# afombravo/2FAST2Q

Hardware: AMD Instinct MI355X
Metric: Mreads/sec matched (150 bp, 20 bp feature, m=1) (higher is better)
Workload: dtype u64 (2-bit packed bases) / u8 qualities

## Files before the change

### 2fast2q_amd/csrc/f2q_count_kernels.h

```cpp
#pragma once

#define F2Q_HIST_MAX 24576u
#define F2Q_HIST_RANGE 38912u

__device__ __forceinline__ unsigned long long wave_sum(unsigned long long v)
{
    for (int o = 32; o > 0; o >>= 1) v += __shfl_down(v, o, 64);
    return v;
}

__device__ __forceinline__ void flush_stats(const Accum &acc, unsigned long long st[5], unsigned long long *lds8,
                                            unsigned long long *slab_row)
{
    const uint32_t lane = threadIdx.x & 63u;
    if (threadIdx.x < 8) lds8[threadIdx.x] = 0;
    __syncthreads();
    for (int k = 0; k < 5; k++) {
        unsigned long long v = wave_sum(st[k]);
        if (lane == 0 && v) atomicAdd(&lds8[k], v);
    }
    __syncthreads();
    if (threadIdx.x < 5) {
        unsigned long long v = lds8[threadIdx.x];
        if (slab_row) gpw(slab_row)[threadIdx.x] = v;
// ... 426 lines not shown
    typedef uint32_t v2 __attribute__((ext_vector_type(2)));
    const v2 v = *reinterpret_cast<const v2 *>(p);
    return U2{v.x, v.y};
}

__device__ __forceinline__ uint32_t lt_count_inc(uint32_t slot) { return 1u << ((slot & 1u) << 4); }
__device__ __forceinline__ uint32_t lt_count_add(uint32_t *cnt, uint32_t bucket, uint32_t inc)
{
    return atomicAdd(&cnt[bucket], inc);
}
__device__ __forceinline__ bool lt_count_passed(uint32_t old, uint32_t inc) { return ((old >> (inc >> 12)) & 0xFFFFu) == 0x7FFFu; }
__device__ __forceinline__ bool lt_count_maybe_passed(uint32_t old_or) { return (old_or & 0x40004000u) != 0u; }
__device__ __forceinline__ void lt_count_handoff(uint32_t *cnt, uint32_t bucket, uint32_t inc, const Accum &acc, const LtDesc &lt)
{
    atomicSub(&cnt[bucket], inc << 15);
    acc_add(&acc.counts[gp(lt.feat_of)[2u * bucket + (inc >> 16)]], 0x8000ull);
}
__device__ __forceinline__ void lt_count(uint32_t *cnt, uint32_t slot, const Accum &acc, const LtDesc &lt)
{
    const uint32_t bucket = slot >> 1, inc = lt_count_inc(slot);
    if (lt_count_passed(lt_count_add(cnt, bucket, inc), inc)) lt_count_handoff(cnt, bucket, inc, acc, lt);
}

template <int NQ, int NB, bool NEAR, bool A20, bool MW = false>
__global__ __launch_bounds__(F2Q_LT_THREADS) void k_count_fixed4_lds(const RunDev *__restrict__ runp,
                                                                     const LibDev *__restrict__ libp, PackedBlock pb,
                                                                     Accum acc)
{
    extern __shared__ uint32_t lt_smem[];
    constexpr uint32_t NT = NEAR ? 2u : 1u;
    uint32_t *tg = lt_smem;
// ... 1149 lines not shown
    __syncthreads();
    typedef uint32_t v4 __attribute__((ext_vector_type(4)));
    const uint64_t n4 = n_slots / 4;
    const auto hb = (const v4 F2Q_GLOBAL *)hit_buf;
    for (uint64_t i = (uint64_t)part * 1024u + threadIdx.x; i < n4; i += (uint64_t)n_parts * 1024u) {
        const v4 v = hb[i];
        const uint32_t e[4] = {v.x - f0, v.y - f0, v.z - f0, v.w - f0};
#pragma unroll
        for (int k = 0; k < 4; k++) if (e[k] < fn) atomicAdd(&rh[e[k]], 1u);
    }
    __syncthreads();
    auto row = (uint32_t F2Q_GLOBAL *)slab + (uint64_t)part * nf + f0;
    for (uint32_t i = threadIdx.x; i < fn; i += 1024u) row[i] = rh[i];
}

#define F2Q_RED_SPLIT 8u
__global__ __launch_bounds__(256) void k_reduce_slabs(const uint32_t *__restrict__ slab, uint32_t n_rows, uint32_t nf,
                                                       unsigned long long *__restrict__ counts,
                                                       const unsigned long long *__restrict__ stat_slab, uint32_t n_stat_rows,
                                                       unsigned long long *__restrict__ stats)
{
    __shared__ unsigned long long part[256];
    if (blockIdx.x == 0 && blockIdx.y == 0 && stat_slab) {
        const uint32_t k = threadIdx.x & 7u, sub = threadIdx.x >> 3;
        unsigned long long sv = 0;
        if (k < 5) for (uint32_t w = sub; w < n_stat_rows; w += 32u) sv += stat_slab[(uint64_t)w * 8u + k];
        part[threadIdx.x] = sv;
        __syncthreads();
        if (threadIdx.x < 5) {
            unsigned long long tot = 0;
            for (uint32_t q = 0; q < 32u; q++) tot += part[q * 8u + threadIdx.x];
            if (tot) atomicAdd(&stats[threadIdx.x], tot);
        }
        __syncthreads();
    }
    const uint32_t fx = threadIdx.x & 63u, ry = threadIdx.x >> 6;
    const uint32_t f = blockIdx.x * 64u + fx;
    unsigned long long sum = 0;
    if (f < nf) {
        const uint32_t step = F2Q_RED_SPLIT * 4u;
#pragma unroll 8
        for (uint32_t w = blockIdx.y * 4u + ry; w < n_rows; w += step) sum += slab[(uint64_t)w * nf + f];
    }
    part[threadIdx.x] = sum;
    __syncthreads();
    if (ry == 0 && f < nf) {
        sum = part[fx] + part[64 + fx] + part[128 + fx] + part[192 + fx];
        if (sum) atomicAdd(&counts[f], sum);
    }
}

struct RawBlock {
    uint64_t n;
    uint64_t first_index;
    const uint8_t *raw;
    const unsigned long long *off;
    const unsigned long long *qoff;
    const uint32_t *len, *qlen, *index;
    const uint32_t *len1, *qlen1;
    const unsigned long long *hdr_umi;
};

#define F2Q_GEN_THREADS 64
// ... 46 lines not shown
```

### 2fast2q_amd/csrc/f2q_device.h

```cpp
#pragma once
#include <stdint.h>

#ifndef F2Q_HD
#ifdef __HIPCC__
#define F2Q_HD __host__ __device__ __forceinline__
#else
#define F2Q_HD inline
#endif
#endif

#define F2Q_DEV_MAX_ITER 16
#define F2Q_ANCHOR_MAX 128
#define F2Q_MAX_PIECES 8
#define F2Q_REG_MAXLEN 31
#define F2Q_TILE 256
#define F2Q_LEN_SKIP 0xFFFFu
#define F2Q_LEN_FLAG 0x8000u
#define F2Q_LEN_CASE 0x4000u
#define F2Q_LEN_MASK 0x3FFFu

namespace f2q {

#if defined(__HIP_DEVICE_COMPILE__)
#define F2Q_GLOBAL __attribute__((address_space(1)))
// ... 100 lines not shown
    const uint64_t *tab_keys;
    const uint32_t *tab_idx;
    const uint8_t *feat_bytes;
    const uint32_t *feat_off;
    const uint32_t *irr_ids;
    LenGroup grp[F2Q_REG_MAXLEN + 1];
};

struct Accum {
    unsigned long long *counts;
    unsigned long long *stats;
    uint32_t *slab;
    unsigned long long *stat_slab;
    unsigned long long *stamp;
    uint32_t *hit_buf;
};

struct EcDev {
    unsigned long long *slots;
    uint32_t mask;
    uint32_t max_entries;
    unsigned long long *ent_off;
    uint32_t *ent_len;
    unsigned long long *ent_count;
    unsigned long long *ent_first;
    uint32_t *arena;
    unsigned long long arena_words;
    unsigned long long *ctr;
    unsigned long long *k64_slots;
    unsigned long long *k64_count;
// ... 2484 lines not shown
```

### 2fast2q_amd/csrc/f2q_lib.hip

```cpp
#include <hip/hip_runtime.h>
#include <stdio.h>
#include <stdlib.h>
#include <string.h>
#include <zlib.h>

#include <algorithm>
#include <atomic>
#include <string>
#include <chrono>
#include <condition_variable>
#include <deque>
#include <functional>
#include <map>
#include <memory>
#include <unordered_map>
#include <mutex>
#include <thread>
#include <vector>

#include "f2q_device.h"
#include "f2q_host.h"
#include "f2q_synth.h"
#include "f2q_reader.h"

// ... 33 lines not shown
    RunDev *run_d = nullptr;
    PackPlan plan{};
    int n_mate1 = 0;
    bool rc2 = false;
    bool have_lib = false;
    HostIndex ix;
    LibDev lib_h{};
    LibDev *lib_d = nullptr;
    std::vector<void *> lib_allocs;
    uint64_t *guide_keys_d = nullptr;
    std::vector<uint64_t> synth_keys;
    uint64_t *synth_keys_d = nullptr;
    uint32_t synth_glen = 0;
    unsigned long long *acc_d = nullptr;
    uint64_t acc_n = 0;
    uint32_t *slab_d = nullptr;
    size_t slab_n = 0;
    unsigned long long *stat_slab_d = nullptr;
    size_t stat_slab_n = 0;
    uint32_t *hit_buf_d = nullptr;
    size_t hit_buf_n = 0;
    EcDev ec{};
    std::vector<void *> ec_allocs;
    std::vector<void *> ec_allocs64;
    std::vector<void *> ec_allocs_ctr;
    hipStream_t aux_stream = nullptr;
    hipEvent_t ev_aux0 = nullptr, ev_aux1 = nullptr;
    bool aux_busy = false;
    uint64_t ec_slots = 0;
    EcHot hot{};
// ... 247 lines not shown
        L.gk.fw = gk_fw; L.gk.fwoff = gk_fwoff;
    }
    L.tab_keys = tk; L.tab_idx = ti; L.feat_bytes = fb; L.feat_off = fo; L.irr_ids = ir;
    if (guide_keys) *guide_keys = gk;
    LibDev *ld;
    if ((rc = dev_upload(c, &L, 1, &ld, owner))) return rc;
    *lib_d = ld;
    HIPC(c, hipStreamSynchronize(c->stream));
    return F2Q_OK;
}
static int upload_lib(f2q_ctx *c) { return upload_index(c, c->ix, c->lib_h, &c->lib_d, c->lib_allocs, &c->guide_keys_d); }

static int alloc_acc(f2q_ctx *c, uint64_t n_features)
{
    if (c->acc_d) { (void)hipFree(c->acc_d); c->acc_d = nullptr; }
    c->acc_n = n_features + 5;
    HIPC(c, hipMalloc((void **)&c->acc_d, c->acc_n * sizeof(unsigned long long)));
    HIPC(c, hipMemsetAsync(c->acc_d, 0, c->acc_n * sizeof(unsigned long long), c->stream));
    HIPC(c, hipStreamSynchronize(c->stream));
    return F2Q_OK;
}

extern "C" int f2q_create(const f2q_params *p, f2q_ctx **out)
{
    if (!p || !out) return fail(nullptr, F2Q_EINVAL, "null argument");
    *out = nullptr;
    int ndev = 0;
    hipError_t e = hipGetDeviceCount(&ndev);
    if (e != hipSuccess || ndev < 1)
        return fail(nullptr, F2Q_ENODEVICE, std::string("no HIP device: ") + hipGetErrorString(e));
    if (p->device < 0 || p->device >= ndev) return fail(nullptr, F2Q_EINVAL, "device ordinal out of range");
    if (p->mode != 0 && p->mode != 1) return fail(nullptr, F2Q_EINVAL, "mode must be 0 (C) or 1 (EC)");
    f2q_ctx *c = new f2q_ctx();
    c->prm = *p;
// ... 191 lines not shown
    if (c->aux_stream) (void)hipStreamSynchronize(c->aux_stream);
    free_all(c, c->lib_allocs); free_all(c, c->ec_allocs); free_all(c, c->ec_allocs64); free_all(c, c->ec_allocs_ctr); free_all(c, c->hot_allocs);
    free_all(c, c->asg_lib_allocs); free_all(c, c->asg_allocs);
    if (c->trace && c->umi.on) fprintf(stderr, "[f2q trace] UMI set: %llu slots, %llu rehashes\n", (unsigned long long)c->umi.n_slots, (unsigned long long)c->umi.rehashes);
    umi_drop(c);
    demux_drop(c);
    strand_drop(c);
    if (c->trace && c->parts.on) fprintf(stderr, "[f2q trace] recombinant set: %llu slots, %llu rehashes\n", (unsigned long long)c->parts.n_slots, (unsigned long long)c->parts.rehashes);
    parts_drop(c);
    free_all(c, c->stagger.allocs);
    if (c->asg_acc_d) (void)hipFree(c->asg_acc_d);
    if (c->defer_d) (void)hipFree(c->defer_d);
    for (auto &kv : c->dev_idle) (void)hipFree(kv.second);
    c->dev_idle.clear(); c->dev_size.clear();
    if (c->acc_d) (void)hipFree(c->acc_d);
    if (c->synth_keys_d) (void)hipFree(c->synth_keys_d);
    if (c->slab_d) (void)hipFree(c->slab_d);
    if (c->stat_slab_d) (void)hipFree(c->stat_slab_d);
    if (c->hit_buf_d) (void)hipFree(c->hit_buf_d);
    if (c->pt_s.streams) (void)hipFree(c->pt_s.streams);
    if (c->pt_s.cnt) (void)hipFree(c->pt_s.cnt);
    if (c->pt_stat_d) (void)hipFree(c->pt_stat_d);
    if (c->pt_slab0_d) (void)hipFree(c->pt_slab0_d);
    if (c->pt_slab1_d) (void)hipFree(c->pt_slab1_d);
    if (c->run_d) (void)hipFree(c->run_d);
    if (c->ev_a) (void)hipEventDestroy(c->ev_a);
    if (c->ev_b) (void)hipEventDestroy(c->ev_b);
    if (c->ev_k0) (void)hipEventDestroy(c->ev_k0);
    if (c->ev_k1) (void)hipEventDestroy(c->ev_k1);
    for (hipEvent_t e : c->q_ev) (void)hipEventDestroy(e);
// ... 37 lines not shown
    if (c->demux.on) { demux_drop(c); if ((rc = demux_alloc(c))) return rc; }
    if (c->strand.mode) { strand_drop(c); if ((rc = strand_alloc(c))) return rc; }
    if (c->parts.on && (rc = parts_install(c, seqs ? seqs : "", offs, n))) return rc;
    if (c->stagger.n) HIPC(c, hipMemsetAsync(c->stagger.dev.hist, 0, 2 * ((size_t)c->stagger.n + 1) * sizeof(unsigned long long), c->stream));
    c->plan.inband_n = (c->plan.fast_fixed || c->plan.fast_anchor) && c->ix.n_irregular == 0;
    if (c->plan.fast_anchor && c->plan.multi_pair && c->prm.mode == 0 && c->run_h.n_iter == 2 && c->lib_h.pw.ok) { c->plan.inband_n = true; c->plan.n_only = true; }
    if (c->ix.n_irregular && !c->plan.multi_pair) c->plan.fast_anchor = false;
    c->have_lib = true;
    return F2Q_OK;
}

extern "C" int f2q_reset_counts(f2q_ctx *c)
{
    if (!c) return F2Q_EINVAL;
    HIPC(c, hipSetDevice(c->device));
    HIPC(c, hipMemsetAsync(c->acc_d, 0, c->acc_n * sizeof(unsigned long long), c->stream));
    if (c->prm.mode == 1) {
        if (c->aux_stream) HIPC(c, hipStreamSynchronize(c->aux_stream));
        c->aux_busy = false;
        free_all(c, c->ec_allocs); free_all(c, c->ec_allocs64); free_all(c, c->ec_allocs_ctr);
        memset(&c->ec, 0, sizeof c->ec); c->ec_slots = 0; c->hot_valid = false; c->ec_learned = 0;
    }
    if (c->umi.on && c->umi.dev.umis) if (int rc = umi_clear(c)) return rc;
    if (c->demux.on && c->demux.dev.matrix) if (int rc = demux_clear(c)) return rc;
    if (c->strand.mode && c->strand.dev.rev_counts) HIPC(c, hipMemsetAsync(c->strand.dev.rev_counts, 0, c->strand.words * sizeof(unsigned long long), c->stream));
    if (c->parts.on && c->parts.dev.counts) if (int rc = parts_clear(c)) return rc;
    if (c->stagger.n) HIPC(c, hipMemsetAsync(c->stagger.dev.hist, 0, 2 * ((size_t)c->stagger.n + 1) * sizeof(unsigned long long), c->stream));
    c->reads_seen = 0;
    c->ec_gen++;
    return F2Q_OK;
}

extern "C" int f2q_set_read_base(f2q_ctx *c, uint64_t first_read_index)
{
    if (!c) return F2Q_EINVAL;
    c->reads_seen = first_read_index;
    return F2Q_OK;
}

extern "C" int f2q_read_counts(f2q_ctx *c, int64_t *counts, int64_t stats[5])
{
    if (!c) return F2Q_EINVAL;
    HIPC(c, hipSetDevice(c->device));
    std::vector<unsigned long long> h(c->acc_n);
    HIPC(c, hipMemcpyAsync(h.data(), c->acc_d, c->acc_n * sizeof(unsigned long long), hipMemcpyDeviceToHost, c->stream));
    HIPC(c, hipStreamSynchronize(c->stream));
    if (counts) for (uint64_t i = 0; i + 5 < c->acc_n; i++) counts[i] = (int64_t)h[i];
    if (stats) for (int k = 0; k < 5; k++) stats[k] = (int64_t)h[c->acc_n - 5 + k];
    return F2Q_OK;
}

extern "C" int f2q_counts_device_ptr(f2q_ctx *c, void **dptr, uint64_t *n_int64)
{
    if (!c || !dptr || !n_int64) return F2Q_EINVAL;
    *dptr = c->acc_d; *n_int64 = c->acc_n;
    return F2Q_OK;
}

static const char *const STAGGER_NO_UMI = "a stagger context (f2q_set_stagger) takes no UMIs: the two are not combined";
static const char *const STRAND_NO_UMI = "a context with a strand mode (f2q_set_strand: rev / both) takes no UMIs: the two are not combined";
static const char *const PARTS_NO_UMI = "a parts context (f2q_set_parts) takes no UMIs: the two are not combined";
static const char *const DEMUX_NO_UMI = "a demultiplexing context (f2q_set_sample_barcodes) takes no UMIs: the two are not combined";
static void umi_enable(f2q_ctx *c)
{
    c->umi.on = true;
    { const char *e = getenv("F2Q_UMI_SLOTS"); if (e && atol(e) > 0) { c->umi.min_slots = 2; while (c->umi.min_slots < (uint64_t)atol(e) && c->umi.min_slots < (1ull << 32)) c->umi.min_slots <<= 1; } }
    c->force_general = true;
    c->plan.fast_fixed = false; c->plan.fast_anchor = false; c->plan.multi = false; c->plan.multi_pair = false;
    c->plan.inband_n = false; c->plan.n_only = false;
// ... 443 lines not shown
    if (zero) HIPC(c, hipMemsetAsync(*buf, 0, want * sizeof(T), c->stream));
    have = want;
    return F2Q_OK;
}
static int slab_rows(f2q_ctx *c, size_t rows, size_t stat_rows, Accum &acc)
{
    int rc;
    if ((rc = grow_buf(c, &c->slab_d, c->slab_n, std::max<size_t>(rows * c->lib_h.n_features, 1), false))) return rc;
    if ((rc = grow_buf(c, &c->stat_slab_d, c->stat_slab_n, stat_rows * 8, false))) return rc;
    acc.slab = c->slab_d; acc.stat_slab = c->stat_slab_d;
    return F2Q_OK;
}
static int reduce_slabs(f2q_ctx *c, const Accum &acc, uint32_t rows, uint32_t stat_rows, uint32_t &launches)
{
    const uint32_t nf = c->lib_h.n_features;
    hipLaunchKernelGGL(k_reduce_slabs, dim3(std::max<uint32_t>(1u, (nf + 63) / 64), F2Q_RED_SPLIT), dim3(256), 0, c->stream,
                       c->slab_d, rows, nf, acc.counts, c->stat_slab_d, stat_rows, acc.stats);
    HIPC(c, hipGetLastError());
    launches++;
    return F2Q_OK;
}
static bool same_q(const RunDev &r) { return r.thr_up == r.thr && r.thr_down == r.thr; }

template <int N> using int_c = std::integral_constant<int, N>;
template <bool WIDE = false, class F>
static void anchored_geom(int nw, int kb, bool sameq, F &&f)
{
    if constexpr (WIDE) {
        if (nw == 10) return f(int_c<10>(), int_c<3>(), std::false_type());
    }
    auto by_kb = [&](auto NW) {
        auto by_sq = [&](auto KB) { if (sameq) f(NW, KB, std::true_type()); else f(NW, KB, std::false_type()); };
        if (kb == 0) by_sq(int_c<0>()); else if (kb == 1) by_sq(int_c<1>()); else by_sq(int_c<3>());
    };
// ... 66 lines not shown
    launches++;
    return lds && nf ? reduce_slabs(c, acc, grid, grid, launches) : F2Q_OK;
}

static int launch_anchor_lds(f2q_ctx *c, const PackedBlock &pb, Accum &acc, uint32_t &launches)
{
    const uint32_t groups = (pb.n_tiles + F2Q_ALT_GROUPS - 1) / F2Q_ALT_GROUPS;
    uint32_t grid = std::min<uint32_t>(groups, (uint32_t)c->n_cu);
    if (c->lt_max_wgs) grid = std::min<uint32_t>(grid, c->lt_max_wgs);
    const bool near = c->run_h.miss > 0;
    const size_t shmem = ((near ? 2u : 1u) * (size_t)F2Q_LT_SLOTS + F2Q_LT_BUCKETS) * 4;
    int rc = slab_rows(c, grid, grid, acc);
    if (rc) return rc;
    anchored_geom(pb.planar_nw, c->plan.kb, true, [&](auto NW, auto KB, auto) {
        auto kern = near ? k_count_anchor_lt<NW, KB, true, true> : k_count_anchor_lt<NW, KB, true, false>;
        (void)hipFuncSetAttribute((const void *)kern, hipFuncAttributeMaxDynamicSharedMemorySize, (int)shmem);
        hipLaunchKernelGGL(kern, dim3(grid), dim3(F2Q_ALT_THREADS), shmem, c->stream, c->run_d, c->lib_d, pb, acc);
    });
    HIPC(c, hipGetLastError());
    launches++;
    return reduce_slabs(c, acc, grid, grid, launches);
}

static int launch_extract_fixed(f2q_ctx *c, const PackedBlock &pb, Accum &acc, uint32_t &launches)
{
    const uint32_t wgs = (pb.n_tiles + F2Q_V2_WAVES - 1) / F2Q_V2_WAVES;
    const uint32_t grid = std::min<uint32_t>(wgs, (uint32_t)c->n_cu * 4u);
    hipLaunchKernelGGL(k_extract_fixed4, dim3(grid), dim3(F2Q_V2_THREADS), 0, c->stream, c->run_d, c->ec, pb, acc, c->reads_seen);
    HIPC(c, hipGetLastError());
    launches++;
    return F2Q_OK;
}

// ... 33 lines not shown
    int rc;
    if ((rc = grow_buf(c, &c->pt_s.streams, c->pt_streams_n, (size_t)grid1 * P * cap, false))) return rc;
    if ((rc = grow_buf(c, &c->pt_s.cnt, c->pt_cnt_n, (size_t)grid1 * P, false))) return rc;
    if ((rc = grow_buf(c, &c->pt_slab0_d, c->pt_slab0_n, (size_t)grid2 * std::max<uint32_t>(pt.max_part, 1u), true))) return rc;
    if ((rc = grow_buf(c, &c->pt_slab1_d, c->pt_slab1_n, (size_t)n_slots1, true))) return rc;
    if ((rc = grow_buf(c, &c->pt_stat_d, c->pt_stat_n, (size_t)rows * 8, true))) return rc;
    PartScratch ps = c->pt_s;
    ps.cap = cap; ps.n_wg1 = grid1;
    Accum a1 = acc, a2 = acc;
    a1.stat_slab = c->pt_stat_d; a2.stat_slab = a1.stat_slab + (size_t)grid1 * 8;
    const FixedVariant fv = fixed_variant(c, fixed_geom(c->run_h));
    const bool near = c->run_h.miss > 0;
    const size_t shmem1 = (size_t)pw * P * F2Q_PS_RING * 8 + (size_t)(pw + 1) * P * 4;
    const size_t shmem2 = ((size_t)F2Q_LT_SLOTS + F2Q_LT_BUCKETS) * 4 + (near ? (size_t)cw * (F2Q_PC_RING * 8 + F2Q_PC_VIA * 4) : 0);
    auto kern2 = near ? k_part_count<true> : k_part_count<false>;
    (void)hipFuncSetAttribute((const void *)kern2, hipFuncAttributeMaxDynamicSharedMemorySize, (int)shmem2);
    for (uint32_t t0 = 0; t0 < pb.n_tiles; t0 += chunk_tiles) {
        const uint32_t t1 = std::min<uint32_t>(pb.n_tiles, t0 + chunk_tiles);
        auto scatter = [&](auto PW) {
            auto k1 = fv == FV_A20 ? k_part_scatter<5, 2, true, PW> : fv == FV_SPEC52 ? k_part_scatter<5, 2, false, PW> : k_part_scatter<0, 0, false, PW>;
            (void)hipFuncSetAttribute((const void *)k1, hipFuncAttributeMaxDynamicSharedMemorySize, (int)shmem1);
            hipLaunchKernelGGL(k1, dim3(grid1), dim3(64 * PW), shmem1, c->stream, c->run_d, c->lib_d, pb, a1, ps, t0, t1);
        };
        if (pw == 16) scatter(int_c<16>()); else if (pw == 8) scatter(int_c<8>()); else scatter(int_c<4>());
        HIPC(c, hipGetLastError());
        hipLaunchKernelGGL(kern2, dim3(grid2), dim3(64 * cw), shmem2, c->stream, c->run_d, c->lib_d, a2, ps, c->pt_slab0_d, c->pt_slab1_d);
        HIPC(c, hipGetLastError());
        launches += 2;
    }
    hipLaunchKernelGGL(k_part_reduce, dim3(std::max<uint32_t>(1u, (nf + 63) / 64)), dim3(256), 0, c->stream, c->lib_d, c->pt_slab0_d, K,
                       near ? c->pt_slab1_d : (uint32_t *)nullptr, acc.counts, c->pt_stat_d, rows, acc.stats);
    HIPC(c, hipGetLastError());
    launches++;
    return F2Q_OK;
}

template <bool MW>
static auto fixed_lds_kernel(bool near, FixedVariant fv)
{
    if (near) return fv == FV_A20 ? k_count_fixed4_lds<5, 2, true, true, MW> : fv == FV_SPEC52 ? k_count_fixed4_lds<5, 2, true, false, MW> : k_count_fixed4_lds<0, 0, true, false, MW>;
    return fv == FV_A20 ? k_count_fixed4_lds<5, 2, false, true, MW> : fv == FV_SPEC52 ? k_count_fixed4_lds<5, 2, false, false, MW> : k_count_fixed4_lds<0, 0, false, false, MW>;
}
static int launch_fixed_lds(f2q_ctx *c, const PackedBlock &pb, Accum &acc, uint32_t &launches, bool mw)
{
    const uint32_t wgs = (pb.n_tiles + F2Q_LT_WAVES - 1) / F2Q_LT_WAVES;
    const uint32_t grid = std::min<uint32_t>(wgs, c->lt_max_wgs ? std::min<uint32_t>(c->lt_max_wgs, (uint32_t)c->n_cu) : (uint32_t)c->n_cu);
    const bool near = c->run_h.miss > 0;
    const size_t shmem = ((near ? 2u : 1u) * (size_t)F2Q_LT_SLOTS + F2Q_LT_BUCKETS) * 4;
    const FixedVariant fv = fixed_variant(c, mw ? fixed_geom_at(0, c->run_h.n_iter * c->run_h.length, c->run_h.thr) : fixed_geom(c->run_h));
    auto kern = mw ? fixed_lds_kernel<true>(near, fv) : fixed_lds_kernel<false>(near, fv);
    int rc = slab_rows(c, grid, grid, acc);
    if (rc) return rc;
    (void)hipFuncSetAttribute((const void *)kern, hipFuncAttributeMaxDynamicSharedMemorySize, (int)shmem);
    hipLaunchKernelGGL(kern, dim3(grid), dim3(F2Q_LT_THREADS), shmem, c->stream, c->run_d, c->lib_d, pb, acc);
    HIPC(c, hipGetLastError());
    launches++;
    return reduce_slabs(c, acc, grid, grid, launches);
}

static int launch_fixed_packed(f2q_ctx *c, const PackedBlock &pb, Accum &acc, uint32_t &launches)
{
    const uint32_t nf = c->lib_h.n_features;
    const bool lds = nf <= F2Q_HIST_MAX;
    const uint32_t wgs = (pb.n_tiles + F2Q_V2_WAVES - 1) / F2Q_V2_WAVES;
    uint32_t grid = std::min<uint32_t>(wgs, (uint32_t)c->n_cu * 2u);
    if (c->lt_max_wgs) grid = std::min<uint32_t>(grid, c->lt_max_wgs);
    const size_t shmem = (size_t)F2Q_V2_WAVES * F2Q_V2_QCAP * 12 + (lds ? (size_t)nf * 4 : (size_t)F2Q_V2_WAVES * F2Q_V2_QCAP * 4);
    const bool spec52 = fixed_variant(c, fixed_geom(c->run_h)) != FV_GENERIC;
    auto kern = lds ? (spec52 ? k_count_fixed4<true, 5, 2> : k_count_fixed4<true, 0, 0>)
                    : (spec52 ? k_count_fixed4<false, 5, 2> : k_count_fixed4<false, 0, 0>);
    const uint32_t n_ranges = lds ? 1u : (nf + F2Q_HIST_RANGE - 1) / F2Q_HIST_RANGE;
    const uint32_t n_parts = lds ? grid : std::max<uint32_t>(1u, (uint32_t)c->n_cu / n_ranges);
    int rc = slab_rows(c, n_parts, grid, acc);
    if (rc) return rc;
    if (!lds) {
        if ((rc = grow_buf(c, &c->hit_buf_d, c->hit_buf_n, pb.n_slots, false))) return rc;
        acc.hit_buf = c->hit_buf_d;
    }
    hipLaunchKernelGGL(kern, dim3(grid), dim3(F2Q_V2_THREADS), shmem, c->stream, c->run_d, c->lib_d, pb, acc);
    HIPC(c, hipGetLastError());
    launches++;
    if (!lds && nf) {
        (void)hipFuncSetAttribute((const void *)k_hist_ranges, hipFuncAttributeMaxDynamicSharedMemorySize, (int)(F2Q_HIST_RANGE * 4));
        hipLaunchKernelGGL(k_hist_ranges, dim3(n_ranges * n_parts), dim3(1024), (size_t)F2Q_HIST_RANGE * 4, c->stream,
                           c->hit_buf_d, (uint64_t)pb.n_slots, nf, n_parts, c->slab_d);
        HIPC(c, hipGetLastError());
        launches++;
    }
    return nf ? reduce_slabs(c, acc, n_parts, grid, launches) : F2Q_OK;
}

static int launch_fixed_v1(f2q_ctx *c, const PackedBlock &pb, Accum &acc, uint32_t &launches)
{
    const uint32_t grid = std::min<uint32_t>(pb.n_tiles, (uint32_t)c->n_cu * 8u);
    if (c->lib_h.n_features <= F2Q_HIST_MAX) {
        const size_t shmem = std::max<size_t>(4, (size_t)c->lib_h.n_features * 4);
        hipLaunchKernelGGL(k_count_fixed<true>, dim3(grid), dim3(F2Q_TILE), shmem, c->stream, c->run_d, c->lib_d, pb, acc);
    } else {
// ... 216 lines not shown
    uint64_t occupied = 0;
    for (uint64_t i = 0; i < c->umi.n_slots; i++) if (words[i] != KEY_EMPTY && occupied++ < *n) held.emplace_back(words[i], cnt[i]);
    if (occupied != *n) return fail(c, F2Q_EHIP, "the UMI set holds " + std::to_string(occupied) + " pairs, its counter says " + std::to_string(*n));
    std::sort(held.begin(), held.end());
    for (size_t i = 0; i < held.size(); i++) {
        if (feature) feature[i] = (uint32_t)(held[i].first >> 32);
        if (codes) codes[i] = (uint32_t)held[i].first;
        if (reads) reads[i] = held[i].second;
    }
    return F2Q_OK;
}

static int launch_view(f2q_ctx *c, const PackedBlock &pb, const RawBlock &rbv, Accum &acc, uint32_t &launches)
{
    int rc = F2Q_OK;
    if (pb.n_tiles) switch (c->last_path = choose_path(c, pb)) {
        case F2Q_PATH_PAIRS:        rc = launch_pairs(c, pb, acc, launches); break;
        case F2Q_PATH_ANCHOR:       rc = launch_anchor(c, pb, acc, launches); break;
        case F2Q_PATH_ANCHOR_LDS:   rc = launch_anchor_lds(c, pb, acc, launches); break;
        case F2Q_PATH_EXTRACT:      rc = pb.planar_nw ? launch_anchor(c, pb, acc, launches) : launch_extract_fixed(c, pb, acc, launches); break;
        case F2Q_PATH_MULTI_LDS:    rc = launch_fixed_lds(c, pb, acc, launches, true); break;
        case F2Q_PATH_MULTI:        rc = launch_multi(c, pb, acc, launches); break;
        case F2Q_PATH_FIXED_PART:   rc = launch_part(c, pb, acc, launches); break;
        case F2Q_PATH_FIXED_LDS:    rc = launch_fixed_lds(c, pb, acc, launches, false); break;
        case F2Q_PATH_FIXED_PACKED: rc = launch_fixed_packed(c, pb, acc, launches); break;
        default:                    rc = launch_fixed_v1(c, pb, acc, launches); break;
    }
    if (rc || !rbv.n) return rc;
    RawBlock rb = rbv;
    rb.first_index += c->reads_seen;
    const uint64_t wg = (rb.n + F2Q_GEN_THREADS - 1) / F2Q_GEN_THREADS;
    const uint32_t grid = (uint32_t)std::min<uint64_t>(wg, (uint64_t)c->n_cu * 64u);
    if (c->umi.on) {
        if ((rc = umi_reserve(c, rb.n))) return rc;
        if (c->umi.hdr_sep) {
            if (!rb.hdr_umi) return fail(c, F2Q_ESTATE, "a block without header UMIs on a header-UMI context");
            const bool keep = c->umi.dev.reads != nullptr;
#define F2Q_LAUNCH_UMI_HDR(...) hipLaunchKernelGGL((__VA_ARGS__), dim3(grid), dim3(F2Q_GEN_THREADS), 0, c->stream, c->run_d, c->lib_d, c->ec, rb, acc, c->umi.dev)
            if (!rb.len1) { if (keep) F2Q_LAUNCH_UMI_HDR(k_count_umi<true, true>); else F2Q_LAUNCH_UMI_HDR(k_count_umi<false, true>); }
            else if (keep) F2Q_LAUNCH_UMI_HDR(k_count_umi_pair<true, F2Q_UMI_PAIR_STAGE_DEFAULT, true>);
            else F2Q_LAUNCH_UMI_HDR(k_count_umi_pair<false, F2Q_UMI_PAIR_STAGE_DEFAULT, true>);
#undef F2Q_LAUNCH_UMI_HDR
        }
// ... 114 lines not shown
}

static int launch_hot(f2q_ctx *c, const PackedBlock &v, uint64_t slot_base, Accum &acc, uint32_t &launches, bool learning,
                      unsigned long long ctr[F2Q_CTR_WORDS], const f2q_block *aux_block)
{
    int rc = hot_arrays(c);
    if (rc) return rc;
    c->last_path = F2Q_PATH_EXTRACT;
    if (learning) HIPC(c, hipMemsetAsync(c->hot.keys, 0xFF, (size_t)F2Q_HOT_SLOTS * 8, c->stream));
    const size_t shmem = (size_t)F2Q_HOT_SLOTS * 12;
    if (!v.planar_nw) {
        const uint32_t wgs = (v.n_tiles + F2Q_FH_WAVES - 1) / F2Q_FH_WAVES;
        uint32_t fgrid = std::min<uint32_t>(wgs, (uint32_t)c->n_cu);
        if (c->lt_max_wgs) fgrid = std::min<uint32_t>(fgrid, c->lt_max_wgs);
        auto kern = learning ? k_extract_fixed4_hot<true> : k_extract_fixed4_hot<false>;
        (void)hipFuncSetAttribute((const void *)kern, hipFuncAttributeMaxDynamicSharedMemorySize, (int)shmem);
        hipLaunchKernelGGL(kern, dim3(fgrid), dim3(F2Q_FH_THREADS), shmem, c->stream, c->run_d, c->ec, c->hot, v, acc, c->reads_seen,
                           c->defer_d, slot_base, (uint64_t)c->defer_cap);
    } else {
        const uint32_t groups = (v.n_tiles + F2Q_HOT_GROUPS - 1) / F2Q_HOT_GROUPS;
        uint32_t grid = std::min<uint32_t>(groups, (uint32_t)c->n_cu);
        if (c->lt_max_wgs) grid = std::min<uint32_t>(grid, c->lt_max_wgs);
        anchored_geom(v.planar_nw, c->plan.kb, same_q(c->run_h), [&](auto NW, auto KB, auto SQ) {
            auto kern = learning ? k_extract_anchor_hot<NW, KB, SQ, true> : k_extract_anchor_hot<NW, KB, SQ, false>;
            (void)hipFuncSetAttribute((const void *)kern, hipFuncAttributeMaxDynamicSharedMemorySize, (int)shmem);
            hipLaunchKernelGGL(kern, dim3(grid), dim3(F2Q_HOT_THREADS), shmem, c->stream, c->run_d, c->ec, c->hot, v, acc,
                               c->reads_seen, c->defer_d, slot_base, (uint64_t)c->defer_cap);
        });
    }
    HIPC(c, hipGetLastError());
    launches++;
    if (aux_block && (rc = launch_aux_general(c, aux_block, acc, launches))) return rc;
    EC_POINT(c, learning ? "k_extract_anchor_hot (learning)" : "k_extract_anchor_hot");
    return ec_counters(c, ctr);
}

static int hot_aside(f2q_ctx *c, const PackedBlock &blk, Accum &acc, uint32_t &launches, const unsigned long long ctr[F2Q_CTR_WORDS])
{
    const unsigned long long n_def = ctr[F2Q_CTR_ASIDE], n_slow = ctr[F2Q_CTR_ASIDE_SLOW];
    if (!n_def) return F2Q_OK;
    const unsigned long long *known = ctr;
    if (c->aux_busy) { HIPC(c, hipStreamSynchronize(c->aux_stream)); c->aux_busy = false; known = nullptr; }
    int rc = ec_reserve(c, n_slow, n_def, n_def * ((uint64_t)blk.rmax + F2Q_MAX_ITER), known);
// ... 19 lines not shown
    return F2Q_OK;
}

static int launch_block(f2q_ctx *c, const f2q_block *b, f2q_timing *t, hipEvent_t k0 = nullptr, hipEvent_t k1 = nullptr)
{
    if (!k0) { k0 = c->ev_k0; k1 = c->ev_k1; }
    if (c->prm.mode == 0 && !c->have_lib) return fail(c, F2Q_ESTATE, "f2q_set_features must be called before counting in Counter mode");
    if (c->umi.on && b->pb.n_tiles) return fail(c, F2Q_ESTATE, "the block was packed before f2q_set_umi: a UMI context counts raw records only");
    if (c->stagger.n && (b->pb.n_tiles || b->rb.len1)) return fail(c, F2Q_ESTATE, "the block was packed before f2q_set_stagger: a stagger context counts single raw records only");
    if (c->strand.mode && (b->pb.n_tiles || b->rb.len1)) return fail(c, F2Q_ESTATE, "the block was packed before f2q_set_strand: a context with a strand mode counts single raw records only");
    if (c->demux.on && (b->pb.n_tiles || b->rb.len1)) return fail(c, F2Q_ESTATE, "the block was packed before f2q_set_sample_barcodes: a demultiplexing context counts single raw records only");
    if (c->parts.on && (b->pb.n_tiles || (b->rb.n && (b->rb.len1 != nullptr) != (c->n_mate1 != 0))))
        return fail(c, F2Q_ESTATE, "the block was packed before f2q_set_parts: a parts context counts raw records only");
    if (c->umi.hdr_sep && b->rb.n && !b->rb.hdr_umi) return fail(c, F2Q_ESTATE, "the block was made before f2q_set_umi_header (or without headers): its records carry no header UMI");
    c->counted = true;
    Accum acc{c->acc_d, c->acc_d + (c->acc_n - 5), nullptr, nullptr, nullptr, nullptr};
#ifdef F2Q_STAMP
    static unsigned long long *stamp_d = nullptr;
    if (!stamp_d) { (void)hipMalloc((void **)&stamp_d, 64); (void)hipMemset(stamp_d, 0, 64); }
    acc.stamp = stamp_d;
#endif
    uint32_t launches = 0;
    HIPC(c, hipEventRecord(k0, c->stream));
    c->ec_gen++;
    if (c->prm.mode == 0) {
        int rc = launch_view(c, b->pb, b->rb, acc, launches);
        if (rc) return rc;
    } else if (b->n_reads) {
        uint64_t step = (uint64_t)8 << 20;
        { const char *e = getenv("F2Q_EC_STEP"); if (e && atol(e) >= F2Q_TILE) step = (uint64_t)atol(e); }
        const uint32_t tiles_per = (uint32_t)std::max<uint64_t>(1, step / F2Q_TILE);
        const RawBlock none{};
        auto view_of = [&](uint32_t t0, uint32_t nt) {
            PackedBlock v = b->pb;
            v.n_tiles = nt; v.n_slots = (uint64_t)nt * F2Q_TILE;
            v.bases += (size_t)t0 * v.wb * F2Q_TILE; v.qual += (size_t)t0 * v.wq * F2Q_TILE;
            if (v.len) v.len += (size_t)t0 * F2Q_TILE;
            if (v.index) v.index += (size_t)t0 * F2Q_TILE; else v.first_index += (uint64_t)t0 * F2Q_TILE;
            return v;
        };
        const bool hot_path = ec_hot_path(c, b);
        if (hot_path) {
            const uint64_t n = (uint64_t)b->pb.n_tiles * F2Q_TILE;
// ... 1699 lines not shown
        const uint32_t grid = (uint32_t)std::min<uint64_t>((nb + F2Q_ASG_THREADS - 1) / F2Q_ASG_THREADS, (uint64_t)c->n_cu * 8u);
        hipLaunchKernelGGL(k_assign_entries, dim3(grid), dim3(F2Q_ASG_THREADS), 0, c->stream, c->run_d, c->asg_lib_d, c->ec, c->asg,
                           (unsigned long long)nb, ctr[1], st_d);
        HIPC(c, hipGetLastError());
        launches++;
        EC_POINT(c, "k_assign_entries");
    }
    if (nw && ctr[3]) {
        const uint32_t grid = (uint32_t)std::min<uint64_t>((nw + F2Q_ASG_THREADS - 1) / F2Q_ASG_THREADS, (uint64_t)c->n_cu * 8u);
        hipLaunchKernelGGL(k_assign_slots, dim3(grid), dim3(F2Q_ASG_THREADS), 0, c->stream, c->run_d, c->asg_lib_d, c->ec, c->asg, st_d);
        HIPC(c, hipGetLastError());
        launches++;
        EC_POINT(c, "k_assign_slots");
    }
    HIPC(c, hipEventRecord(c->ev_k1, c->stream));
    HIPC(c, hipMemcpyAsync(st_d + F2Q_READS, c->acc_d + (c->acc_n - 5) + F2Q_READS, 8, hipMemcpyDeviceToDevice, c->stream));
    HIPC(c, hipMemcpyAsync(st_d + F2Q_QUALITY_FAILED, c->acc_d + (c->acc_n - 5) + F2Q_QUALITY_FAILED, 8, hipMemcpyDeviceToDevice, c->stream));
    std::vector<unsigned long long> h(nf + 6);
    HIPC(c, hipMemcpyAsync(h.data(), c->asg_acc_d, (nf + 6) * sizeof(unsigned long long), hipMemcpyDeviceToHost, c->stream));
    HIPC(c, hipStreamSynchronize(c->stream));
    if (h[nf + 5]) return fail(c, F2Q_ESTATE, std::to_string(h[nf + 5]) + " Extract+Count entries are not filled in");
    if (counts) for (uint64_t i = 0; i < nf; i++) counts[i] = (int64_t)h[i];
    if (stats) for (int k = 0; k < 5; k++) stats[k] = (int64_t)h[nf + k];
    if (t) {
        float ms = 0;
        HIPC(c, hipEventElapsedTime(&ms, c->ev_k0, c->ev_k1));
        t->kernel_ms = ms; t->total_ms = ms; t->reads = h[nf + F2Q_READS]; t->launches = launches;
    }
    c->asg_nb = nb; c->asg_nw = ctr[3] ? nw : 0; c->asg_gen = c->ec_gen;
    return F2Q_OK;
// ... 31 lines not shown
```

Baseline: 182,600.

## Defer accumulator reset into slab reduction and vectorize reduce kernel

Removes the per-reset memset of the counts accumulator by marking it pending and having the slab-reduction kernel store rather than add on the first reduce; other paths clear it lazily. Overflow handoffs from the LDS counters go to a separate carry buffer that the reduce folds in and clears. The reduce kernel now uses one block per 64 features with 16-row unrolled vector loads instead of a 2D grid with atomics. hipFuncSetAttribute calls are cached per device and kernel to cut host overhead. This adds state-tracking complexity and relies on the store flag being correct on every path.

```diff
diff --git a/2fast2q_amd/csrc/f2q_count_kernels.h b/2fast2q_amd/csrc/f2q_count_kernels.h
--- a/2fast2q_amd/csrc/f2q_count_kernels.h
+++ b/2fast2q_amd/csrc/f2q_count_kernels.h
@@ -464,7 +464,7 @@
 __device__ __forceinline__ void lt_count_handoff(uint32_t *cnt, uint32_t bucket, uint32_t inc, const Accum &acc, const LtDesc &lt)
 {
     atomicSub(&cnt[bucket], inc << 15);
-    acc_add(&acc.counts[gp(lt.feat_of)[2u * bucket + (inc >> 16)]], 0x8000ull);
+    acc_add(&acc.carry[gp(lt.feat_of)[2u * bucket + (inc >> 16)]], 0x8000ull);
 }
 __device__ __forceinline__ void lt_count(uint32_t *cnt, uint32_t slot, const Accum &acc, const LtDesc &lt)
 {
@@ -1644,39 +1644,81 @@
     for (uint32_t i = threadIdx.x; i < fn; i += 1024u) row[i] = rh[i];
 }
 
-#define F2Q_RED_SPLIT 8u
+#define F2Q_RED_FEATS 64u
 __global__ __launch_bounds__(256) void k_reduce_slabs(const uint32_t *__restrict__ slab, uint32_t n_rows, uint32_t nf,
-                                                       unsigned long long *__restrict__ counts,
+                                                       unsigned long long *__restrict__ counts, unsigned long long *__restrict__ carry,
                                                        const unsigned long long *__restrict__ stat_slab, uint32_t n_stat_rows,
-                                                       unsigned long long *__restrict__ stats)
-{
-    __shared__ unsigned long long part[256];
-    if (blockIdx.x == 0 && blockIdx.y == 0 && stat_slab) {
+                                                       unsigned long long *__restrict__ stats, uint32_t store)
+{
+    __shared__ unsigned long long part[16][F2Q_RED_FEATS];
+    if (blockIdx.x == gridDim.x - 1u) {
         const uint32_t k = threadIdx.x & 7u, sub = threadIdx.x >> 3;
         unsigned long long sv = 0;
-        if (k < 5) for (uint32_t w = sub; w < n_stat_rows; w += 32u) sv += stat_slab[(uint64_t)w * 8u + k];
-        part[threadIdx.x] = sv;
+        if (k < 5)
+#pragma unroll 8
+            for (uint32_t w = sub; w < n_stat_rows; w += 32u) sv += gp(stat_slab)[(uint64_t)w * 8u + k];
+        (&part[0][0])[threadIdx.x] = sv;
         __syncthreads();
         if (threadIdx.x < 5) {
             unsigned long long tot = 0;
-            for (uint32_t q = 0; q < 32u; q++) tot += part[q * 8u + threadIdx.x];
-            if (tot) atomicAdd(&stats[threadIdx.x], tot);
-        }
-        __syncthreads();
-    }
-    const uint32_t fx = threadIdx.x & 63u, ry = threadIdx.x >> 6;
-    const uint32_t f = blockIdx.x * 64u + fx;
-    unsigned long long sum = 0;
-    if (f < nf) {
-        const uint32_t step = F2Q_RED_SPLIT * 4u;
-#pragma unroll 8
-        for (uint32_t w = blockIdx.y * 4u + ry; w < n_rows; w += step) sum += slab[(uint64_t)w * nf + f];
-    }
-    part[threadIdx.x] = sum;
-    __syncthreads();
-    if (ry == 0 && f < nf) {
-        sum = part[fx] + part[64 + fx] + part[128 + fx] + part[192 + fx];
-        if (sum) atomicAdd(&counts[f], sum);
+            for (uint32_t q = 0; q < 32u; q++) tot += (&part[0][0])[q * 8u + threadIdx.x];
+            if (store) gpw(stats)[threadIdx.x] = tot;
+            else if (tot) gpw(stats)[threadIdx.x] += tot;
+        }
+        return;
+    }
+    typedef uint32_t v4 __attribute__((ext_vector_type(4)));
+    constexpr uint32_t R = 16u;
+    const uint32_t col = threadIdx.x & 15u, rl = threadIdx.x >> 4;
+    const uint32_t fb = blockIdx.x * F2Q_RED_FEATS, last_row = n_rows - 1u;
+    const bool wide = (nf & 3u) == 0u;
+    unsigned long long s[4] = {0, 0, 0, 0};
+    if (wide && fb + 4u * col < nf) {
+        const auto p = gp(slab) + (fb + 4u * col);
+        for (uint32_t w0 = rl; w0 < n_rows; w0 += 16u * R) {
+            v4 v[R];
+#pragma unroll
+            for (uint32_t i = 0; i < R; i++) v[i] = *reinterpret_cast<const v4 F2Q_GLOBAL *>(p + (uint64_t)min(w0 + 16u * i, last_row) * nf);
+            __builtin_amdgcn_sched_barrier(0);
+#pragma unroll
+            for (uint32_t i = 0; i < R; i++) {
+                const bool live = w0 + 16u * i < n_rows;
+                s[0] += live ? v[i].x : 0u; s[1] += live ? v[i].y : 0u; s[2] += live ? v[i].z : 0u; s[3] += live ? v[i].w : 0u;
+            }
+        }
+    } else if (!wide) {
+        uint32_t fk[4];
+#pragma unroll
+        for (uint32_t k = 0; k < 4u; k++) fk[k] = min(fb + col + 16u * k, nf - 1u);
+        for (uint32_t w0 = rl; w0 < n_rows; w0 += 16u * R) {
+            uint32_t v[R][4];
+#pragma unroll
+            for (uint32_t i = 0; i < R; i++) {
+                const auto row = gp(slab) + (uint64_t)min(w0 + 16u * i, last_row) * nf;
+#pragma unroll
+                for (uint32_t k = 0; k < 4u; k++) v[i][k] = row[fk[k]];
+            }
+            __builtin_amdgcn_sched_barrier(0);
+#pragma unroll
+            for (uint32_t i = 0; i < R; i++) {
+                const bool live = w0 + 16u * i < n_rows;
+#pragma unroll
+                for (uint32_t k = 0; k < 4u; k++) s[k] += live ? v[i][k] : 0u;
+            }
+        }
+    }
+#pragma unroll
+    for (uint32_t k = 0; k < 4u; k++) part[rl][wide ? 4u * col + k : col + 16u * k] = s[k];
+    __syncthreads();
+    const uint32_t f = blockIdx.x * F2Q_RED_FEATS + threadIdx.x;
+    if (threadIdx.x < F2Q_RED_FEATS && f < nf) {
+        unsigned long long sum = 0;
+#pragma unroll
+        for (uint32_t r = 0; r < 16u; r++) sum += part[r][threadIdx.x];
+        const unsigned long long cv = gp(carry)[f];
+        if (cv) { gpw(carry)[f] = 0; sum += cv; }
+        if (store) gpw(counts)[f] = sum;
+        else if (sum) gpw(counts)[f] += sum;
     }
 }
 
diff --git a/2fast2q_amd/csrc/f2q_device.h b/2fast2q_amd/csrc/f2q_device.h
--- a/2fast2q_amd/csrc/f2q_device.h
+++ b/2fast2q_amd/csrc/f2q_device.h
@@ -138,6 +138,7 @@
     unsigned long long *stat_slab;
     unsigned long long *stamp;
     uint32_t *hit_buf;
+    unsigned long long *carry;
 };
 
 struct EcDev {
diff --git a/2fast2q_amd/csrc/f2q_lib.hip b/2fast2q_amd/csrc/f2q_lib.hip
--- a/2fast2q_amd/csrc/f2q_lib.hip
+++ b/2fast2q_amd/csrc/f2q_lib.hip
@@ -71,6 +71,8 @@
     uint32_t synth_glen = 0;
     unsigned long long *acc_d = nullptr;
     uint64_t acc_n = 0;
+    bool acc_pending = false, acc_eager = false;
+    unsigned long long *carry_d = nullptr;
     uint32_t *slab_d = nullptr;
     size_t slab_n = 0;
     unsigned long long *stat_slab_d = nullptr;
@@ -348,10 +350,23 @@
 static int alloc_acc(f2q_ctx *c, uint64_t n_features)
 {
     if (c->acc_d) { (void)hipFree(c->acc_d); c->acc_d = nullptr; }
+    if (c->carry_d) { (void)hipFree(c->carry_d); c->carry_d = nullptr; }
     c->acc_n = n_features + 5;
+    const size_t carry_n = (size_t)std::max<uint64_t>(n_features, 1);
     HIPC(c, hipMalloc((void **)&c->acc_d, c->acc_n * sizeof(unsigned long long)));
+    HIPC(c, hipMalloc((void **)&c->carry_d, carry_n * sizeof(unsigned long long)));
     HIPC(c, hipMemsetAsync(c->acc_d, 0, c->acc_n * sizeof(unsigned long long), c->stream));
+    HIPC(c, hipMemsetAsync(c->carry_d, 0, carry_n * sizeof(unsigned long long), c->stream));
     HIPC(c, hipStreamSynchronize(c->stream));
+    c->acc_pending = false;
+    return F2Q_OK;
+}
+
+static int acc_ready(f2q_ctx *c)
+{
+    if (!c->acc_pending) return F2Q_OK;
+    HIPC(c, hipMemsetAsync(c->acc_d, 0, c->acc_n * sizeof(unsigned long long), c->stream));
+    c->acc_pending = false;
     return F2Q_OK;
 }
 
@@ -573,6 +588,7 @@
     for (auto &kv : c->dev_idle) (void)hipFree(kv.second);
     c->dev_idle.clear(); c->dev_size.clear();
     if (c->acc_d) (void)hipFree(c->acc_d);
+    if (c->carry_d) (void)hipFree(c->carry_d);
     if (c->synth_keys_d) (void)hipFree(c->synth_keys_d);
     if (c->slab_d) (void)hipFree(c->slab_d);
     if (c->stat_slab_d) (void)hipFree(c->stat_slab_d);
@@ -640,7 +656,8 @@
 {
     if (!c) return F2Q_EINVAL;
     HIPC(c, hipSetDevice(c->device));
-    HIPC(c, hipMemsetAsync(c->acc_d, 0, c->acc_n * sizeof(unsigned long long), c->stream));
+    c->acc_pending = true;
+    if (c->acc_eager) if (int rc = acc_ready(c)) return rc;
     if (c->prm.mode == 1) {
         if (c->aux_stream) HIPC(c, hipStreamSynchronize(c->aux_stream));
         c->aux_busy = false;
@@ -668,6 +685,7 @@
 {
     if (!c) return F2Q_EINVAL;
     HIPC(c, hipSetDevice(c->device));
+    if (int rc = acc_ready(c)) return rc;
     std::vector<unsigned long long> h(c->acc_n);
     HIPC(c, hipMemcpyAsync(h.data(), c->acc_d, c->acc_n * sizeof(unsigned long long), hipMemcpyDeviceToHost, c->stream));
     HIPC(c, hipStreamSynchronize(c->stream));
@@ -679,6 +697,9 @@
 extern "C" int f2q_counts_device_ptr(f2q_ctx *c, void **dptr, uint64_t *n_int64)
 {
     if (!c || !dptr || !n_int64) return F2Q_EINVAL;
+    HIPC(c, hipSetDevice(c->device));
+    if (int rc = acc_ready(c)) return rc;
+    c->acc_eager = true;
     *dptr = c->acc_d; *n_int64 = c->acc_n;
     return F2Q_OK;
 }
@@ -1152,10 +1173,23 @@
 static int reduce_slabs(f2q_ctx *c, const Accum &acc, uint32_t rows, uint32_t stat_rows, uint32_t &launches)
 {
     const uint32_t nf = c->lib_h.n_features;
-    hipLaunchKernelGGL(k_reduce_slabs, dim3(std::max<uint32_t>(1u, (nf + 63) / 64), F2Q_RED_SPLIT), dim3(256), 0, c->stream,
-                       c->slab_d, rows, nf, acc.counts, c->stat_slab_d, stat_rows, acc.stats);
+    const uint32_t store = c->acc_pending ? 1u : 0u;
+    hipLaunchKernelGGL(k_reduce_slabs, dim3((nf + F2Q_RED_FEATS - 1) / F2Q_RED_FEATS + 1u), dim3(256), 0, c->stream,
+                       c->slab_d, rows, nf, acc.counts, acc.carry, c->stat_slab_d, stat_rows, acc.stats, store);
     HIPC(c, hipGetLastError());
+    c->acc_pending = false;
     launches++;
+    return F2Q_OK;
+}
+static int dyn_lds(f2q_ctx *c, const void *kern, size_t shmem)
+{
+    static std::mutex mu;
+    static std::map<std::pair<int, const void *>, size_t> set;
+    std::lock_guard<std::mutex> lock(mu);
+    size_t &have = set[{c->device, kern}];
+    if (shmem <= have) return F2Q_OK;
+    HIPC(c, hipFuncSetAttribute(kern, hipFuncAttributeMaxDynamicSharedMemorySize, (int)shmem));
+    have = shmem;
     return F2Q_OK;
 }
 static bool same_q(const RunDev &r) { return r.thr_up == r.thr && r.thr_down == r.thr; }
@@ -1252,9 +1286,10 @@
     if (rc) return rc;
     anchored_geom(pb.planar_nw, c->plan.kb, true, [&](auto NW, auto KB, auto) {
         auto kern = near ? k_count_anchor_lt<NW, KB, true, true> : k_count_anchor_lt<NW, KB, true, false>;
-        (void)hipFuncSetAttribute((const void *)kern, hipFuncAttributeMaxDynamicSharedMemorySize, (int)shmem);
+        if ((rc = dyn_lds(c, (const void *)kern, shmem))) return;
         hipLaunchKernelGGL(kern, dim3(grid), dim3(F2Q_ALT_THREADS), shmem, c->stream, c->run_d, c->lib_d, pb, acc);
     });
+    if (rc) return rc;
     HIPC(c, hipGetLastError());
     launches++;
     return reduce_slabs(c, acc, grid, grid, launches);
@@ -1318,15 +1353,16 @@
     const size_t shmem1 = (size_t)pw * P * F2Q_PS_RING * 8 + (size_t)(pw + 1) * P * 4;
     const size_t shmem2 = ((size_t)F2Q_LT_SLOTS + F2Q_LT_BUCKETS) * 4 + (near ? (size_t)cw * (F2Q_PC_RING * 8 + F2Q_PC_VIA * 4) : 0);
     auto kern2 = near ? k_part_count<true> : k_part_count<false>;
-    (void)hipFuncSetAttribute((const void *)kern2, hipFuncAttributeMaxDynamicSharedMemorySize, (int)shmem2);
+    if ((rc = dyn_lds(c, (const void *)kern2, shmem2))) return rc;
     for (uint32_t t0 = 0; t0 < pb.n_tiles; t0 += chunk_tiles) {
         const uint32_t t1 = std::min<uint32_t>(pb.n_tiles, t0 + chunk_tiles);
         auto scatter = [&](auto PW) {
             auto k1 = fv == FV_A20 ? k_part_scatter<5, 2, true, PW> : fv == FV_SPEC52 ? k_part_scatter<5, 2, false, PW> : k_part_scatter<0, 0, false, PW>;
-            (void)hipFuncSetAttribute((const void *)k1, hipFuncAttributeMaxDynamicSharedMemorySize, (int)shmem1);
+            if ((rc = dyn_lds(c, (const void *)k1, shmem1))) return;
             hipLaunchKernelGGL(k1, dim3(grid1), dim3(64 * PW), shmem1, c->stream, c->run_d, c->lib_d, pb, a1, ps, t0, t1);
         };
         if (pw == 16) scatter(int_c<16>()); else if (pw == 8) scatter(int_c<8>()); else scatter(int_c<4>());
+        if (rc) return rc;
         HIPC(c, hipGetLastError());
         hipLaunchKernelGGL(kern2, dim3(grid2), dim3(64 * cw), shmem2, c->stream, c->run_d, c->lib_d, a2, ps, c->pt_slab0_d, c->pt_slab1_d);
         HIPC(c, hipGetLastError());
@@ -1355,7 +1391,7 @@
     auto kern = mw ? fixed_lds_kernel<true>(near, fv) : fixed_lds_kernel<false>(near, fv);
     int rc = slab_rows(c, grid, grid, acc);
     if (rc) return rc;
-    (void)hipFuncSetAttribute((const void *)kern, hipFuncAttributeMaxDynamicSharedMemorySize, (int)shmem);
+    if ((rc = dyn_lds(c, (const void *)kern, shmem))) return rc;
     hipLaunchKernelGGL(kern, dim3(grid), dim3(F2Q_LT_THREADS), shmem, c->stream, c->run_d, c->lib_d, pb, acc);
     HIPC(c, hipGetLastError());
     launches++;
@@ -1385,7 +1421,7 @@
     HIPC(c, hipGetLastError());
     launches++;
     if (!lds && nf) {
-        (void)hipFuncSetAttribute((const void *)k_hist_ranges, hipFuncAttributeMaxDynamicSharedMemorySize, (int)(F2Q_HIST_RANGE * 4));
+        if ((rc = dyn_lds(c, (const void *)k_hist_ranges, (size_t)F2Q_HIST_RANGE * 4))) return rc;
         hipLaunchKernelGGL(k_hist_ranges, dim3(n_ranges * n_parts), dim3(1024), (size_t)F2Q_HIST_RANGE * 4, c->stream,
                            c->hit_buf_d, (uint64_t)pb.n_slots, nf, n_parts, c->slab_d);
         HIPC(c, hipGetLastError());
@@ -1632,7 +1668,13 @@
 static int launch_view(f2q_ctx *c, const PackedBlock &pb, const RawBlock &rbv, Accum &acc, uint32_t &launches)
 {
     int rc = F2Q_OK;
-    if (pb.n_tiles) switch (c->last_path = choose_path(c, pb)) {
+    if (pb.n_tiles) {
+        c->last_path = choose_path(c, pb);
+        const bool slab_only = c->prm.mode == 0 && c->lib_h.n_features &&
+                               (c->last_path == F2Q_PATH_FIXED_LDS || c->last_path == F2Q_PATH_MULTI_LDS || c->last_path == F2Q_PATH_FIXED_PACKED);
+        if (!slab_only && (rc = acc_ready(c))) return rc;
+    }
+    if (pb.n_tiles) switch (c->last_path) {
         case F2Q_PATH_PAIRS:        rc = launch_pairs(c, pb, acc, launches); break;
         case F2Q_PATH_ANCHOR:       rc = launch_anchor(c, pb, acc, launches); break;
         case F2Q_PATH_ANCHOR_LDS:   rc = launch_anchor_lds(c, pb, acc, launches); break;
@@ -1645,6 +1687,7 @@
         default:                    rc = launch_fixed_v1(c, pb, acc, launches); break;
     }
     if (rc || !rbv.n) return rc;
+    if ((rc = acc_ready(c))) return rc;
     RawBlock rb = rbv;
     rb.first_index += c->reads_seen;
     const uint64_t wg = (rb.n + F2Q_GEN_THREADS - 1) / F2Q_GEN_THREADS;
@@ -1789,7 +1832,7 @@
         uint32_t fgrid = std::min<uint32_t>(wgs, (uint32_t)c->n_cu);
         if (c->lt_max_wgs) fgrid = std::min<uint32_t>(fgrid, c->lt_max_wgs);
         auto kern = learning ? k_extract_fixed4_hot<true> : k_extract_fixed4_hot<false>;
-        (void)hipFuncSetAttribute((const void *)kern, hipFuncAttributeMaxDynamicSharedMemorySize, (int)shmem);
+        if ((rc = dyn_lds(c, (const void *)kern, shmem))) return rc;
         hipLaunchKernelGGL(kern, dim3(fgrid), dim3(F2Q_FH_THREADS), shmem, c->stream, c->run_d, c->ec, c->hot, v, acc, c->reads_seen,
                            c->defer_d, slot_base, (uint64_t)c->defer_cap);
     } else {
@@ -1798,10 +1841,11 @@
         if (c->lt_max_wgs) grid = std::min<uint32_t>(grid, c->lt_max_wgs);
         anchored_geom(v.planar_nw, c->plan.kb, same_q(c->run_h), [&](auto NW, auto KB, auto SQ) {
             auto kern = learning ? k_extract_anchor_hot<NW, KB, SQ, true> : k_extract_anchor_hot<NW, KB, SQ, false>;
-            (void)hipFuncSetAttribute((const void *)kern, hipFuncAttributeMaxDynamicSharedMemorySize, (int)shmem);
+            if ((rc = dyn_lds(c, (const void *)kern, shmem))) return;
             hipLaunchKernelGGL(kern, dim3(grid), dim3(F2Q_HOT_THREADS), shmem, c->stream, c->run_d, c->ec, c->hot, v, acc,
                                c->reads_seen, c->defer_d, slot_base, (uint64_t)c->defer_cap);
         });
+        if (rc) return rc;
     }
     HIPC(c, hipGetLastError());
     launches++;
@@ -1851,7 +1895,7 @@
         return fail(c, F2Q_ESTATE, "the block was packed before f2q_set_parts: a parts context counts raw records only");
     if (c->umi.hdr_sep && b->rb.n && !b->rb.hdr_umi) return fail(c, F2Q_ESTATE, "the block was made before f2q_set_umi_header (or without headers): its records carry no header UMI");
     c->counted = true;
-    Accum acc{c->acc_d, c->acc_d + (c->acc_n - 5), nullptr, nullptr, nullptr, nullptr};
+    Accum acc{c->acc_d, c->acc_d + (c->acc_n - 5), nullptr, nullptr, nullptr, nullptr, c->carry_d};
 #ifdef F2Q_STAMP
     static unsigned long long *stamp_d = nullptr;
     if (!stamp_d) { (void)hipMalloc((void **)&stamp_d, 64); (void)hipMemset(stamp_d, 0, 64); }
@@ -1864,6 +1908,7 @@
         int rc = launch_view(c, b->pb, b->rb, acc, launches);
         if (rc) return rc;
     } else if (b->n_reads) {
+        if (int rc = acc_ready(c)) return rc;
         uint64_t step = (uint64_t)8 << 20;
         { const char *e = getenv("F2Q_EC_STEP"); if (e && atol(e) >= F2Q_TILE) step = (uint64_t)atol(e); }
         const uint32_t tiles_per = (uint32_t)std::max<uint64_t>(1, step / F2Q_TILE);
@@ -3593,6 +3638,7 @@
         EC_POINT(c, "k_assign_slots");
     }
     HIPC(c, hipEventRecord(c->ev_k1, c->stream));
+    if (int rc = acc_ready(c)) return rc;
     HIPC(c, hipMemcpyAsync(st_d + F2Q_READS, c->acc_d + (c->acc_n - 5) + F2Q_READS, 8, hipMemcpyDeviceToDevice, c->stream));
     HIPC(c, hipMemcpyAsync(st_d + F2Q_QUALITY_FAILED, c->acc_d + (c->acc_n - 5) + F2Q_QUALITY_FAILED, 8, hipMemcpyDeviceToDevice, c->stream));
     std::vector<unsigned long long> h(nf + 6);
```

New measurement: 187,500, median of 6. 1.03x the previous value.
